# ADicksonLab/AGDIFF

Hardware: AMD Instinct MI355X
Metric: conformers/sec (whole node), GEOM-Drugs 5000-step sampling (higher is better)
Workload: dtype f16x3

## Files before the change

agdiff_amd/csrc/edge.hip:

```cpp
#include "common.hpp"

namespace {

__device__ __forceinline__ const lds_u32x4* ag_lds_base(const lds_u32x4* p, int lane) {
  const lds_u32x4* b = p + lane;
  asm volatile("" : "+v"(b));
  return b;
}

struct EncArgs {
  const float* fe_w;
  const float* fe_b;
  const float* t1;
  const float* w1_pk;
  const float* t3;
  const float* w23_pk;
  const float* w4_pk;
  const float* b4;
  const int32_t* n_dev;
  const float* e_len;
  const int32_t* e_type;
  float* out_frag;
  float* out_rows;
  const int32_t* row_index;
// ... 218 lines not shown
    pf_t1 = a.e_dst[last];
  };
  {
    const int64_t first = ((int64_t)wg * AG_CONV_WAVES + wave) * a.chunk_tiles;
    if (first * AG_TW < E) {
#pragma unroll
      for (int t = 0; t < 4; ++t) ag_load_attr(ea[t], a.e_attr, first, t, lane0);
      prefetch_meta(first, lane0);
    }
  }
  for (int64_t chunk = (int64_t)wg * AG_CONV_WAVES + wave; chunk < a.max_chunks; chunk += cstride) {
    const int64_t e_begin = chunk * (AG_TW * a.chunk_tiles);
    if (e_begin >= E) break;
    int run_t = -1;
    float carry[AG_CONV_NCH / 4];
#pragma unroll
    for (int i = 0; i < AG_CONV_NCH / 4; ++i) carry[i] = 0.0f;

    auto dest = [&](int t) -> float* {
      const int lo = a.in_ptr[t];
      return (lo >= e_begin) ? (a.agg + (size_t)t * 192) : (a.agg_first + (size_t)chunk * 192);
    };

    for (int tt = 0; tt < a.chunk_tiles; ++tt) {
      const int64_t tile = chunk * a.chunk_tiles + tt;
      const int64_t tbase = tile * AG_TW;
      if (tbase >= E) break;
      int lane = lane0;
      asm volatile("" : "+v"(lane));
      const int q = lane >> 4, col = lane & 15;
      const int my_src = pf_src;
      const float s1 = pf_s1, s2 = pf_s2;
      const int t0 = __builtin_amdgcn_readfirstlane(pf_t0);
      const int t1 = __builtin_amdgcn_readfirstlane(pf_t1);
      if (run_t >= 0 && run_t != t0) {
        float* dp = dest(run_t);
#pragma unroll
        for (int i = 0; i < AG_CONV_NCH / 4; ++i) {
          dp[16 * (4 * i + q) + col] = carry[i];
          carry[i] = 0.0f;
        }
        run_t = -1;
      }

      uint32_t xoff[4];
      f32x4 sr;
#pragma unroll
      for (int r = 0; r < 4; ++r) {
        xoff[r] = ((uint32_t)__shfl(my_src, 4 * q + r) * 192u + (uint32_t)col) * 4u;
        sr[r] = __shfl(s1, 4 * q + r);
      }
      const int ntg = t1 - t0 + 1;
      const int ipl = a.in_ptr[t0 + (lane <= ntg ? lane : ntg)];
      auto bound = [&](int i) -> int {
        return (i < 64) ? __builtin_amdgcn_readlane(ipl, i) : __builtin_amdgcn_readfirstlane(a.in_ptr[t0 + i]);
      };
      auto dest_lo = [&](int t, int lo) -> float* {
        return (lo >= e_begin) ? (a.agg + (size_t)t * 192) : (a.agg_first + (size_t)chunk * 192);
      };

      constexpr int XA = 2, XR = XA + 1;
      f32x4 xring[XR];
      float bring[XR];
      auto fetch_x = [&](int nt) {
        const char* xb = reinterpret_cast<const char*>(a.xs);
#pragma unroll
        for (int r = 0; r < 4; ++r) xring[nt % XR][r] = *reinterpret_cast<const float*>(xb + (size_t)xoff[r] + 64 * nt);
        bring[nt % XR] = a.cp.filt_b2[16 * nt + col];
      };
#pragma unroll
      for (int nt = 0; nt < XA; ++nt) fetch_x(nt);
      auto prefetch_next = [&]() {
        int64_t nxt = tile + 1;
        if (tt + 1 >= a.chunk_tiles) nxt = (chunk + cstride) * a.chunk_tiles;
        if (nxt * AG_TW < E && nxt < a.max_chunks * a.chunk_tiles) {
#pragma unroll
          for (int t = 0; t < 4; ++t) ag_load_attr(ea[t], a.e_attr, nxt, t, lane);
          prefetch_meta(nxt, lane);
        }
      };
      AgIn<MODE> hidb[6];
      {
        constexpr int WA = 1, WR = WA + 1;
        u32x4 wq[WR][2][2];
        const lds_u32x4* w1_lo = ag_lds_base(w1, lane);
        const lds_u32x4* w1_hi = ag_lds_base(w1 + 32 * 128, lane);
        auto fetch_w = [&](u32x4 (&dst)[2][2], int step) {
          const int m = step >> 2, t = step & 3;
#pragma unroll
          for (int b = 0; b < 2; ++b) {
            const int bi = t * AG_CONV_NCH + 2 * m + b;
            const lds_u32x4* wb = (bi < 32) ? w1_lo + bi * 128 : w1_hi + (bi - 32) * 128;
            dst[b][0] = wb[0];
            dst[b][1] = wb[64];
          }
        };
#pragma unroll
        for (int s0 = 0; s0 < WA; ++s0) fetch_w(wq[s0 % WR], s0);
        f32x4 hp0 = {0.f, 0.f, 0.f, 0.f}, hp1 = {0.f, 0.f, 0.f, 0.f};
#pragma unroll
        for (int m = 0; m <= AG_CONV_NCH / 2; ++m) {
          f32x4 h0 = {0.f, 0.f, 0.f, 0.f}, h1 = {0.f, 0.f, 0.f, 0.f};
          if (m < AG_CONV_NCH / 2) {
            h0 = nb0;
            h1 = nb1;
            const int mn = (m + 1) % (AG_CONV_NCH / 2);
            nb0 = ag_ld4(a.cp.filt_b1 + 32 * mn + 4 * q);
            nb1 = ag_ld4(a.cp.filt_b1 + 32 * mn + 16 + 4 * q);
          }
#pragma unroll
          for (int t = 0; t < 4; ++t) {
            const int step = m * 4 + t;
            if (m < AG_CONV_NCH / 2) {
              if (step + WA < 4 * (AG_CONV_NCH / 2)) fetch_w(wq[(step + WA) % WR], step + WA);
              ag_block_mma<MODE, false>(h0, ea[t], wq[step % WR][0]);
              ag_block_mma<MODE, false>(h1, ea[t], wq[step % WR][1]);
            }
            if (m > 0) {
              float v0 = (t < 2) ? hp0[2 * t] : hp1[2 * t - 4], v1 = (t < 2) ? hp0[2 * t + 1] : hp1[2 * t - 3];
              v0 = ag_ssp_base2(v0); v1 = ag_ssp_base2(v1);
              asm volatile("" : "+v"(v0), "+v"(v1));
              ag_cvt_pair(hidb[m - 1], 2 * t, v0, v1);
            }
            __builtin_amdgcn_sched_barrier(0);
          }
          hp0 = h0; hp1 = h1;
        }
        prefetch_next();
      }
      f32x4 m0, m1;
      {
        const int b0 = bound(0), b1 = bound(1), b2 = bound(ntg >= 2 ? 2 : 1);
#pragma unroll
        for (int r = 0; r < 4; ++r) {
          const int er = (int)tbase + 4 * q + r;
          m0[r] = (er >= b0 && er < b1) ? 1.0f : 0.0f;
          m1[r] = (ntg >= 2 && er >= b1 && er < b2) ? 1.0f : 0.0f;
        }
      }
      float* const dp0 = dest_lo(t0, bound(0));
      const bool fast = ntg <= 2;
      const bool two = ntg == 2;
      auto reduce_general = [&](f32x4 z, int nt, float& cr) {
        const bool mine = q == (nt & 3);
        float newcarry = 0.0f;
        for (int i = 0; i < ntg; ++i) {
          const int lo = bound(i), hi = bound(i + 1);
          float p = 0.0f;
#pragma unroll
          for (int r = 0; r < 4; ++r) {
            const int er = (int)tbase + 4 * q + r;
            p += ((er >= lo) && (er < hi)) ? z[r] : 0.0f;
          }
          p = ag_quarter_sum(p);
          if (i == 0) p = cr + p;
          if (i < ntg - 1) {
            float* dp = dest_lo(t0 + i, lo);
            if (mine) dp[16 * nt + col] = p;
          } else {
            newcarry = p;
          }
        }
        cr = mine ? newcarry : cr;
      };
      const u32x4* gl = reinterpret_cast<const u32x4*>(a.cp.filt_w2b_pk) + lane;
      u32x4 g[2][2];
      auto fetch_g = [&](int pair) {
#pragma unroll
        for (int b = 0; b < 2; ++b) {
          g[b][0] = gl[((2 * pair + b) * 2) * 64];
          g[b][1] = gl[((2 * pair + b) * 2 + 1) * 64];
        }
      };
      const lds_u32x4* w2a_l = ag_lds_base(w2a, lane);
      constexpr int LA = 1, LR = LA + 1;
      u32x4 w2q[LR][2];
      auto fetch_w2 = [&](int b) {
        w2q[b % LR][0] = w2a_l[(b * 2) * 64];
        w2q[b % LR][1] = w2a_l[(b * 2 + 1) * 64];
      };
#pragma unroll
      for (int b = 0; b < LA; ++b) fetch_w2(b);
      auto dense2 = [&](int nt) -> f32x4 {
        f32x4 z[1] = {{0.f, 0.f, 0.f, 0.f}};
        if (nt == 7) fetch_g(0);
        if (nt < 8) {
#pragma unroll
          for (int k = 0; k < 4; ++k) {
            const int b = nt * 4 + k;
            if (b + LA < 32) fetch_w2(b + LA);
            ag_block_mma<MODE, true>(z[0], hidb[k], w2q[b % LR]);
          }
        } else {
          ag_block_mma<MODE, true>(z[0], hidb[4], g[0]);
          ag_block_mma<MODE, true>(z[0], hidb[5], g[1]);
          if (nt + 1 < AG_CONV_NCH) fetch_g(nt + 1 - 8);
        }
        return z[0];
      };
      auto factors = [&](int nt, float& bb, f32x4& m, bool with_scale) {
        if (nt == 8) {
#pragma unroll
          for (int r = 0; r < 4; ++r) sr[r] = __shfl(s2, 4 * q + r);
        }
        bb = bring[nt % XR];
        m = with_scale ? sr * xring[nt % XR] : xring[nt % XR];
        if (nt + XA < AG_CONV_NCH) fetch_x(nt + XA);
      };
      auto run_fast = [&](auto TWO) {
        constexpr bool kTwo = decltype(TWO)::value;
        f32x4 zp = {0.f, 0.f, 0.f, 0.f}, mp = {0.f, 0.f, 0.f, 0.f};
        float bp = 0.0f;
        float p0[4], p1[4] = {0.f, 0.f, 0.f, 0.f};
        f32x4 w0 = m0 * sr, w1 = m1 * sr;
#pragma unroll
        for (int nt = 0; nt <= AG_CONV_NCH; ++nt) {
          f32x4 z = {0.f, 0.f, 0.f, 0.f}, m = {0.f, 0.f, 0.f, 0.f};
          float bb = 0.0f;
          if (nt < AG_CONV_NCH) {
            z = dense2(nt);
            factors(nt, bb, m, false);
          }
          if (nt == 9) { w0 = m0 * sr; w1 = m1 * sr; }
          if (nt > 0) {
            const int j = (nt - 1) & 3, g4 = (nt - 1) >> 2;
            f32x4 t;
#pragma unroll
            for (int r = 0; r < 4; ++r) t[r] = (zp[r] + bp) * mp[r];
            p0[j] = t[0] * w0[0];
#pragma unroll
            for (int r = 1; r < 4; ++r) p0[j] = fmaf(t[r], w0[r], p0[j]);
            if constexpr (kTwo) {
              p1[j] = t[0] * w1[0];
#pragma unroll
              for (int r = 1; r < 4; ++r) p1[j] = fmaf(t[r], w1[r], p1[j]);
            }
            if (j == 3) {
              const float r0 = carry[g4] + ag_quarter_reduce_scatter4(p0[0], p0[1], p0[2], p0[3]);
              if constexpr (kTwo) {
                dp0[16 * (4 * g4 + q) + col] = r0;
                carry[g4] = ag_quarter_reduce_scatter4(p1[0], p1[1], p1[2], p1[3]);
              } else {
                carry[g4] = r0;
              }
            }
          }
          zp = z; mp = m; bp = bb;
        }
      };
      if (fast) {
        if (two) run_fast(std::true_type{});
        else run_fast(std::false_type{});
      } else {
#pragma unroll
        for (int nt = 0; nt < AG_CONV_NCH; ++nt) {
          f32x4 z = dense2(nt), m;
          float bb;
          factors(nt, bb, m, true);
#pragma unroll
          for (int r = 0; r < 4; ++r) z[r] = (z[r] + bb) * m[r];
          reduce_general(z, nt, carry[nt >> 2]);
        }
      }
      run_t = t1;
    }
    if (run_t >= 0) {
      float* dp = dest(run_t);
#pragma unroll
      for (int i = 0; i < AG_CONV_NCH / 4; ++i) dp[16 * (4 * i + (lane0 >> 4)) + (lane0 & 15)] = carry[i];
    }
  }
}

struct HeadArgs {
  agdiff_head_params_t hp;
  const int32_t* n_dev;
  const int32_t* src;
  const int32_t* dst;
  const float* node_h;
  const float* attr_frag;
  const float* attr_rows;
  const int32_t* pos_index;
  const int32_t* mir_index;
  float* out;
  int64_t max_tiles;
};

template <int MODE>
__global__ void __launch_bounds__(64 * AG_PERSIST_WAVES, 4) k_pair_head(HeadArgs a) {
  extern __shared__ u32x4 ag_head_smem[];
  lds_u32x4* lw1 = (lds_u32x4*)ag_head_smem;
  lds_u32x4* lw2 = lw1 + 64 * 128;
  {
    const u32x4* g1 = reinterpret_cast<const u32x4*>(a.hp.w1_pk);
    const u32x4* g2 = reinterpret_cast<const u32x4*>(a.hp.w2_pk);
    ag_copy_lds(lw1, g1, 64 * 128);
    ag_copy_lds(lw2, g2, 16 * 128);
  }
  __syncthreads();
  const int lane0 = ag_lane();
  const int E = *a.n_dev;
  const int64_t stride = (int64_t)gridDim.x * AG_PERSIST_WAVES;
  const int64_t wg = (gridDim.x % 8 == 0) ? (int64_t)(blockIdx.x % 8) * (gridDim.x / 8) + blockIdx.x / 8 : (int64_t)blockIdx.x;
  for (int64_t tile = wg * AG_PERSIST_WAVES + (threadIdx.x >> 6); tile < a.max_tiles; tile += stride) {
    if (tile * AG_TW >= E) break;
    int lane = lane0;
    asm volatile("" : "+v"(lane));
    const int q = lane >> 4;
    const int64_t e = tile * AG_TW + (lane & 15);
    const bool valid = e < E;
    const int s = valid ? a.src[e] : 0, t = valid ? a.dst[e] : 0;
    const int pp = (a.pos_index && valid) ? a.pos_index[e] : 0;

    f32x4 y1[8];
    ag_init_vec<8>(y1, a.hp.b1, q);
    {
      const float* hs = a.node_h + (size_t)ag_piece_row_value(s, lane) * 128;
      const float* ht = a.node_h + (size_t)ag_piece_row_value(t, lane) * 128;
      const int64_t er = tile * AG_TW + (lane >> 2);
      const float* ar = a.attr_rows + (size_t)(er < E ? er : 0) * 128;
      const int to_op = ag_to_operand_addr(lane);
      AgIn<MODE> sl[2];
      f32x4 raw[4];
      auto fetch = [&](f32x4 (&r)[4], AgIn<MODE>& dst, int k) {
        if (k < 4) {
          ag_load_slice_pieces(r[0], r[1], hs, k, lane);
          ag_load_slice_pieces(r[2], r[3], ht, k, lane);
        } else if (a.attr_frag && a.pos_index) {
          ag_load_attr(dst, a.attr_frag, (int64_t)(pp >> 4), k - 4, q * 16 + (pp & 15));
        } else if (a.attr_frag) {
          ag_load_attr(dst, a.attr_frag, tile, k - 4, lane);
        } else {
          ag_load_slice_pieces(r[0], r[1], ar, k - 4, lane);
        }
      };
      auto finish = [&](AgIn<MODE>& dst, const f32x4 (&r)[4], int k) {
        if (k < 4) ag_cvt(ag_permute4(r[0] * r[2], to_op), ag_permute4(r[1] * r[3], to_op), dst);
        else if (!a.attr_frag) ag_cvt(ag_permute4(r[0], to_op), ag_permute4(r[1], to_op), dst);
      };
      fetch(raw, sl[0], 0);
      finish(sl[0], raw, 0);
      const lds_u32x4* lw1_lo = ag_lds_base(lw1, lane);
      const lds_u32x4* lw1_hi = ag_lds_base(lw1 + 32 * 128, lane);
#pragma unroll
      for (int k = 0; k < 8; ++k) {
        if (k + 1 < 8) fetch(raw, sl[(k + 1) & 1], k + 1);
        const lds_u32x4* wk = (k < 4) ? lw1_lo + (k * 8) * 128 : lw1_hi + ((k - 4) * 8) * 128;
        if (k & 1) ag_dense_lds<MODE, false, true, 1, 8, 1, 0>(sl, y1, wk, 0);
        else ag_dense_lds<MODE, false, true, 1, 8, 0, 0>(sl, y1, wk, 0);
        if (k + 1 < 8) finish(sl[(k + 1) & 1], raw, k + 1);
      }
    }
    ag_head_act<8>(y1, a.hp.act);
    f32x4 y2[4];
    ag_init_vec<4>(y2, a.hp.b2, q);
    {
      AgIn<MODE> y1b[4];
      ag_report_range<MODE>(ag_absmax<MODE, 8>(y1, 0.0f), a.hp.range_rows, s, valid);
      ag_cvt_tiles<MODE, 4, 0>(y1, y1b);
      ag_dense_lds<MODE, false, false, 4, 4, 0, 0>(y1b, y2, ag_lds_base(lw2, lane), 0);
    }
    ag_head_act<4>(y2, a.hp.act);
    const float o = ag_dot_vec<4>(y2, a.hp.w3, q) + a.hp.b3;
    if (valid && q == 0) {
      int l2 = lane0;
      asm volatile("" : "+v"(l2));
      const int64_t e2 = tile * AG_TW + (l2 & 15);
      a.out[a.pos_index ? (int64_t)pp : e2] = o;
      const int pm = a.pos_index ? a.mir_index[e2] : -1;
      if (pm >= 0) a.out[pm] = o;
    }
  }
}

struct RadScaleArgs {
  const float* dw[2 * AGDIFF_MAX_CONVS];
  const int32_t* rad_cnt;
  int32_t* rad_src;
  float* rad_len;
  float* out;
  int64_t rpad;
  int32_t n;
  float cutoff;
  int32_t smooth;
};
__global__ void __launch_bounds__(256) k_rad_scales(RadScaleArgs a) {
  __shared__ float seg[2 * AGDIFF_MAX_CONVS * 100];
  for (int i = threadIdx.x; i < a.n * 100; i += blockDim.x) seg[i] = a.dw[i / 100][i % 100];
  __syncthreads();
  const int64_t row = (int64_t)blockIdx.x * blockDim.x + threadIdx.x;
  if (row >= a.rpad) return;
  const int i = (int)(row / AGDIFF_RAD_STRIDE), k = (int)(row - (int64_t)i * AGDIFF_RAD_STRIDE);
  const int cnt = a.rad_cnt[i];
  if (k >= ((cnt + AG_TW - 1) / AG_TW) * AG_TW) return;
  if (k >= cnt) {
    a.rad_src[row] = i;
    a.rad_len[row] = 0.0f;
    for (int c = 0; c < a.n; ++c) a.out[(size_t)c * a.rpad + row] = 0.0f;
    return;
  }
  const float d = a.rad_len[row];
  const float C = cf_envelope(d, a.cutoff, a.smooth);
  for (int c = 0; c < a.n; ++c) a.out[(size_t)c * a.rpad + row] = cf_dist_weight(seg + c * 100, d) * C;
}

__global__ void k_zero_word(int32_t* p) {
  if (threadIdx.x == 0) *p = 0;
}

struct AttrPolyArgs {
  const float* poly_pk;
  const int32_t* type_slot;
  const int32_t* n_dev;
  const float* e_len;
  const int32_t* e_type;
  float* out_rows;
  int32_t* flags;
  int64_t max_tiles;
  int32_t num_slots;
  int32_t far_slots;
  const int32_t* type_far;
  float cutoff;
  float two_over_rc;
  float far_hi;
  float two_over_far;
};

#define AG_ATTRP_WAVES 16
#define AG_ATTRP_MAX_SLOTS 9
template <int MODE>
__global__ void __launch_bounds__(64 * AG_ATTRP_WAVES, AG_ATTRP_WAVES / 4) k_edge_attr_poly(AttrPolyArgs a) {
  extern __shared__ u32x4 ag_attrp_smem[];
  lds_u32x4* wl = (lds_u32x4*)ag_attrp_smem;
  __shared__ int wg_flagged;
  if (threadIdx.x == 0) wg_flagged = 0;
  ag_copy_lds(wl, reinterpret_cast<const u32x4*>(a.poly_pk), (a.num_slots + a.far_slots) * 8 * 128);
  __syncthreads();
  const int lane0 = ag_lane();
  const int E = *a.n_dev;
  const int64_t stride = (int64_t)gridDim.x * AG_ATTRP_WAVES;
  int my_flagged = 0;
  for (int64_t tile = (int64_t)blockIdx.x * AG_ATTRP_WAVES + (threadIdx.x >> 6); tile < a.max_tiles; tile += stride) {
    if (tile * AG_TW >= E) break;
    int lane = lane0;
    asm volatile("" : "+v"(lane));
    const int q = lane >> 4;
    const int64_t e = tile * AG_TW + (lane & 15);
    const bool valid = e < E;
    const float d = valid ? a.e_len[e] : 0.0f;
    const int ety = valid ? a.e_type[e] : 0;
    const int tslot = valid ? a.type_slot[ety] : -1;
    const int fset = (valid && a.far_slots > 0) ? a.type_far[ety] : -1;
    const bool is_nan = (__float_as_uint(d) & 0x7FFFFFFFu) > 0x7F800000u;
    const bool far = d > a.cutoff && d <= a.far_hi && tslot >= 0 && fset >= 0;
    const int slot = far ? fset : tslot;
    const bool hard = valid && (is_nan || d < 0.0f || (d > a.cutoff && !far) || tslot < 0);
    const int hard_rows = (int)(__ballot(hard) & 0xFFFFull);
    if (lane == 0) a.flags[1 + tile] = hard_rows;
    if (hard_rows) ++my_flagged;
    if (hard_rows == (int)(__ballot(valid) & 0xFFFFull)) continue;
    AgIn<MODE> phall[1], ph[1];
    ag_poly_features<MODE, 1>(far ? d - a.cutoff : d, far ? a.two_over_far : a.two_over_rc, q, phall);
    f32x4 y[8];
#pragma unroll
    for (int t = 0; t < 8; ++t) y[t] = f32x4{0.f, 0.f, 0.f, 0.f};
    const lds_u32x4* wl_l = ag_lds_base(wl, lane);
    uint64_t todo = __ballot(slot >= 0 && !hard) & 0xFFFFull;
    while (todo) {
      const int g = __builtin_amdgcn_readlane(slot, (int)__builtin_ctzll(todo));
      const bool in = slot == g && !hard;
      todo &= ~__ballot(in);
      const u32x4 zero = {0u, 0u, 0u, 0u};
      if constexpr (MODE == AG_F32) {
        ph[0].v[0] = in ? phall[0].v[0] : f32x4{0.f, 0.f, 0.f, 0.f};
        ph[0].v[1] = in ? phall[0].v[1] : f32x4{0.f, 0.f, 0.f, 0.f};
      } else {
        ph[0].hi = __builtin_bit_cast(decltype(ph[0].hi), in ? __builtin_bit_cast(u32x4, phall[0].hi) : zero);
        ph[0].lo = __builtin_bit_cast(decltype(ph[0].lo), in ? __builtin_bit_cast(u32x4, phall[0].lo) : zero);
      }
      const lds_u32x4* wg_ = wl_l + (size_t)g * (8 * 128);
      u32x4 w[8][2];
#pragma unroll
      for (int ot = 0; ot < 8; ++ot) {
        w[ot][0] = wg_[(ot * 2) * 64];
        w[ot][1] = wg_[(ot * 2 + 1) * 64];
      }
#pragma unroll
      for (int part = 0; part < AgParts<MODE>::n; ++part) {
#pragma unroll
        for (int ot = 0; ot < 8; ++ot) ag_block_mma_part<MODE, false>(y[ot], ph[0], w[ot], part);
      }
    }
    const bool ok = ag_piece_row_value(valid && !hard, lane) != 0;
    ag_store_row_pieces<8, 0>(y, a.out_rows + (size_t)(tile * AG_TW + (lane >> 2)) * 128, ok, lane);
  }
  if (lane0 == 0 && my_flagged) atomicAdd(&wg_flagged, my_flagged);
  __syncthreads();
  if (threadIdx.x == 0 && wg_flagged) atomicAdd(&a.flags[0], wg_flagged);
}

struct HeadPolyArgs {
  agdiff_head_params_t hp;
  const int32_t* n_dev;
  const int32_t* src;
  const int32_t* dst;
  const float* len;
  const float* node_h;
  const int32_t* pos_index;
  const int32_t* mir_index;
  float* out;
  int64_t max_tiles;
  float two_over_rc;
  const int32_t* seg_tile_live;
};

template <int MODE, int NKT>
__global__ void __launch_bounds__(64 * AG_PERSIST_WAVES, 4) k_pair_head_poly(HeadPolyArgs a) {
  extern __shared__ u32x4 ag_headp_smem[];
  lds_u32x4* lw1 = (lds_u32x4*)ag_headp_smem;
  lds_u32x4* lwp = lw1 + 32 * 128;
  lds_u32x4* lw2 = lwp + 8 * NKT * 128;
  {
    const u32x4* g1 = reinterpret_cast<const u32x4*>(a.hp.w1_pk);
    const u32x4* gp = reinterpret_cast<const u32x4*>(a.hp.attr_poly_pk);
    const u32x4* g2 = reinterpret_cast<const u32x4*>(a.hp.w2_pk);
    ag_copy_lds(lw1, g1, 32 * 128);
    ag_copy_lds(lwp, gp, 8 * NKT * 128);
    ag_copy_lds(lw2, g2, 16 * 128);
  }
  __syncthreads();
  const int lane0 = ag_lane();
  const int E = a.seg_tile_live ? 0 : *a.n_dev;
  const int64_t stride = (int64_t)gridDim.x * AG_PERSIST_WAVES;
  const int64_t wg = (gridDim.x % 8 == 0) ? (int64_t)(blockIdx.x % 8) * (gridDim.x / 8) + blockIdx.x / 8 : (int64_t)blockIdx.x;
  for (int64_t tile = wg * AG_PERSIST_WAVES + (threadIdx.x >> 6); tile < a.max_tiles; tile += stride) {
    int64_t live_end;
    if (a.seg_tile_live) {
      const int live = a.seg_tile_live[tile];
      if (live == 0) continue;
      live_end = tile * AG_TW + live;
    } else {
      live_end = E;
      if (tile * AG_TW >= E) break;
    }
    int lane = lane0;
    asm volatile("" : "+v"(lane));
    const int q = lane >> 4;
    const int64_t e = tile * AG_TW + (lane & 15);
    const bool valid = e < live_end;
    const int s = valid ? a.src[e] : 0, t = valid ? a.dst[e] : 0;
    const float d = valid ? a.len[e] : 0.0f;
    const int64_t pe = a.pos_index ? (valid ? (int64_t)a.pos_index[e] : 0) : e;
    const int64_t pm = (a.pos_index && valid) ? (int64_t)a.mir_index[e] : -1;

    f32x4 y1[8];
    ag_init_vec<8>(y1, a.hp.b1, q);
    {
      const float* hs = a.node_h + (size_t)ag_piece_row_value(s, lane) * 128;
      const float* ht = a.node_h + (size_t)ag_piece_row_value(t, lane) * 128;
      const int to_op = ag_to_operand_addr(lane);
      AgIn<MODE> sl[2];
      f32x4 raw[4];
      auto fetch = [&](f32x4 (&r)[4], int k) {
        ag_load_slice_pieces(r[0], r[1], hs, k, lane);
        ag_load_slice_pieces(r[2], r[3], ht, k, lane);
      };
      auto finish = [&](AgIn<MODE>& dst, const f32x4 (&r)[4]) {
        ag_cvt(ag_permute4(r[0] * r[2], to_op), ag_permute4(r[1] * r[3], to_op), dst);
      };
      fetch(raw, 0);
      finish(sl[0], raw);
      const lds_u32x4* lw1_l = ag_lds_base(lw1, lane);
#pragma unroll
      for (int k = 0; k < 4; ++k) {
        if (k + 1 < 4) fetch(raw, k + 1);
        if (k & 1) ag_dense_lds<MODE, false, true, 1, 8, 1, 0>(sl, y1, lw1_l + (k * 8) * 128, 0);
        else ag_dense_lds<MODE, false, true, 1, 8, 0, 0>(sl, y1, lw1_l + (k * 8) * 128, 0);
        if (k + 1 < 4) finish(sl[(k + 1) & 1], raw);
      }
      AgIn<MODE> ph[NKT];
      ag_poly_features<MODE, NKT>(d, a.two_over_rc, q, ph);
      ag_dense_lds<MODE, false, true, NKT, 8, 0, 0>(ph, y1, ag_lds_base(lwp, lane), 0);
    }
    ag_head_act<8>(y1, a.hp.act);
    f32x4 y2[4];
    ag_init_vec<4>(y2, a.hp.b2, q);
    {
      AgIn<MODE> y1b[4];
      ag_report_range<MODE>(ag_absmax<MODE, 8>(y1, 0.0f), a.hp.range_rows, s, valid);
      ag_cvt_tiles<MODE, 4, 0>(y1, y1b);
      ag_dense_lds<MODE, false, false, 4, 4, 0, 0>(y1b, y2, ag_lds_base(lw2, lane), 0);
    }
    ag_head_act<4>(y2, a.hp.act);
    const float o = ag_dot_vec<4>(y2, a.hp.w3, q) + a.hp.b3;
    if (valid && q == 0) {
      a.out[pe] = o;
      if (pm >= 0) a.out[pm] = o;
    }
  }
}

template <int F>
__global__ void __launch_bounds__(AG_WG) k_cfconv_aggregate(const float* __restrict__ x, const float* __restrict__ W,
                                                            const int32_t* __restrict__ in_ptr,
                                                            const int32_t* __restrict__ src, int64_t n,
                                                            float* __restrict__ out) {
  constexpr int LPE = F / 4;
  constexpr int EPI = 64 / LPE;
  const int lane = ag_lane();
  const int64_t node = (int64_t)blockIdx.x * 4 + ag_wave_in_wg();
  if (node >= n) return;
  const int lo = in_ptr[node], hi = in_ptr[node + 1];
  const int sub = lane / LPE, fl = (lane % LPE) * 4;
  f32x4 acc = {0.f, 0.f, 0.f, 0.f};
  for (int e = lo + sub; e < hi; e += EPI) {
    const f32x4 w = ag_ld4(W + (size_t)e * F + fl);
    const f32x4 xv = ag_ld4(x + (size_t)src[e] * F + fl);
    acc += w * xv;
  }
#pragma unroll
  for (int o = LPE; o < 64; o <<= 1) {
#pragma unroll
    for (int q = 0; q < 4; ++q) acc[q] += __shfl_xor(acc[q], o);
  }
  if (sub == 0) ag_st4(out + (size_t)node * F + fl, acc);
}

}

static thread_local const int32_t* g_enc_tile_flags = nullptr;

extern "C" int agdiff_edge_encoder(const agdiff_params_t* p, const int32_t* n_edges_dev, int64_t max_tiles,
                                   const float* e_len, const int32_t* e_type, float* attr_frag, float* attr_rows,
                                   const int32_t* row_index, const int32_t* pos_index, const int32_t* mir_index,
                                   void* stream) {
  if (!p || !n_edges_dev || !e_len || !e_type || (!attr_frag && !attr_rows) || max_tiles < 0 || (!pos_index != !mir_index))
    return AGDIFF_ERR_ARG;
  if (max_tiles == 0) return AGDIFF_OK;
  if (p->edge_encoder == 1) {
    if (!p->ge_offset || !p->ge_emb) return AGDIFF_ERR_ARG;
    GaussArgs g{p->ge_offset, p->ge_emb, n_edges_dev, e_len, e_type, attr_frag, attr_rows, row_index, pos_index, mir_index,
                max_tiles, p->ge_coeff * 1.44269504088896340736f};
    const dim3 grid((unsigned)((max_tiles + 3) / 4));
    ag_by_mode(p->precision, [&](auto M) { k_edge_gaussian<decltype(M)::value><<<grid, dim3(256), 0, (hipStream_t)stream>>>(g); });
    AG_CHECK_LAUNCH();
    return AGDIFF_OK;
  }
  if (p->edge_encoder != 0) return AGDIFF_ERR_ARG;
  EncArgs a{p->ee_fe_w, p->ee_fe_b, p->ee_t1, p->ee_w1_pk, p->ee_t3, p->ee_w23_pk, p->ee_w4_pk, p->ee_b4,
            n_edges_dev, e_len, e_type, attr_frag, attr_rows, row_index, pos_index, mir_index, max_tiles, g_enc_tile_flags};
  g_enc_tile_flags = nullptr;
  int64_t wgs = (max_tiles + AG_PERSIST_WAVES - 1) / AG_PERSIST_WAVES;
  if (wgs > 256) wgs = 256;
  const size_t smem = (size_t)80 * 2048;
  static std::atomic<uint64_t> attr_done{0};
  if (!ag_allow_big_lds(attr_done, smem, k_edge_encoder<AG_BF3>, k_edge_encoder<AG_F32>, k_edge_encoder<AG_H3>)) return AGDIFF_ERR_LAUNCH;
  ag_by_mode(p->precision, [&](auto M) {
    k_edge_encoder<decltype(M)::value><<<dim3((unsigned)wgs), dim3(64 * AG_PERSIST_WAVES), smem, (hipStream_t)stream>>>(a);
  });
  AG_CHECK_LAUNCH();
  return AGDIFF_OK;
}

namespace {
int launch_edge_scales(const agdiff_params_t* p, const int32_t* n_dev, int64_t max_n, const float* e_len,
                       const int32_t* pos_index, const int32_t* mir_index, float* out, int64_t epad, void* stream,
                       const int32_t* zero_slotted_types = nullptr) {
  if (max_n == 0) return AGDIFF_OK;
  ScaleArgs a;
  a.e_type = zero_slotted_types;
  a.type_slot = zero_slotted_types ? p->poly_type_slot : nullptr;
  for (int k = 0; k < p->num_convs; ++k) {
    a.dw[2 * k] = p->conv[k].dist_seg;
    a.dw[2 * k + 1] = p->conv[k].dist_seg + 100;
  }
  a.n_dev = n_dev;
  a.e_len = e_len;
  a.pos_index = pos_index;
  a.mir_index = mir_index;
  a.out = out;
  a.epad = epad;
  a.n = 2 * p->num_convs;
  a.cutoff = p->cutoff;
  a.smooth = p->smooth;
  k_edge_scales<<<dim3((unsigned)((max_n + 255) / 256)), dim3(256), 0, (hipStream_t)stream>>>(a);
  AG_CHECK_LAUNCH();
  return AGDIFF_OK;
}
}

extern "C" int agdiff_edge_scales(const agdiff_params_t* p, const agdiff_topo_t* topo, const agdiff_ws_t* ws,
                                  int32_t per_canonical_edge, void* stream) {
  if (!p || !topo || !ws || !ws->e_scale || !ws->e_len || !ws->num_edges || p->num_convs > AGDIFF_MAX_CONVS)
    return AGDIFF_ERR_ARG;
  if (per_canonical_edge && (!ws->num_canon || !ws->c_len || !ws->c_pos || !ws->c_mir)) return AGDIFF_ERR_ARG;
  const int64_t epad = ((topo->max_edges + AG_TW - 1) / AG_TW) * AG_TW;
  return launch_edge_scales(p, per_canonical_edge ? ws->num_canon : ws->num_edges, topo->max_edges,
                            per_canonical_edge ? ws->c_len : ws->e_len, per_canonical_edge ? ws->c_pos : nullptr,
                            per_canonical_edge ? ws->c_mir : nullptr, ws->e_scale, epad, stream);
}

extern "C" int agdiff_edge_scales_split(const agdiff_params_t* p, const agdiff_topo_t* topo, const agdiff_ws_t* ws,
                                        int32_t which, void* stream) {
  if (!p || !topo || !ws || p->num_convs > AGDIFF_MAX_CONVS) return AGDIFF_ERR_ARG;
  if (which == 0) {
    if (!ws->r_scale || !ws->rad_len || !ws->rad_src || !ws->rad_cnt) return AGDIFF_ERR_ARG;
    if (topo->num_nodes <= 0) return AGDIFF_OK;
    RadScaleArgs a;
    for (int k = 0; k < p->num_convs; ++k) {
      a.dw[2 * k] = p->conv[k].dist_seg;
      a.dw[2 * k + 1] = p->conv[k].dist_seg + 100;
    }
    a.rad_cnt = ws->rad_cnt;
    a.rad_src = ws->rad_src;
    a.rad_len = ws->rad_len;
    a.out = ws->r_scale;
    a.rpad = topo->num_nodes * (int64_t)AGDIFF_RAD_STRIDE;
    a.n = 2 * p->num_convs;
    a.cutoff = p->cutoff;
    a.smooth = p->smooth;
    k_rad_scales<<<dim3((unsigned)((a.rpad + 255) / 256)), dim3(256), 0, (hipStream_t)stream>>>(a);
    AG_CHECK_LAUNCH();
    return AGDIFF_OK;
  }
  if (!ws->lc_len || !ws->num_local_canon) return AGDIFF_ERR_ARG;
  if (which == 1) {
    if (!ws->l_scale || !topo->lc_ppos || !topo->lc_pmir) return AGDIFF_ERR_ARG;
    return launch_edge_scales(p, ws->num_local_canon, topo->num_local_canon, ws->lc_len, topo->lc_ppos, topo->lc_pmir,
                              ws->l_scale, ((topo->num_local_padded + AG_TW - 1) / AG_TW) * AG_TW, stream,
                              agdiff_local_poly_enabled(p, topo, ws) == 2 ? topo->lc_type : nullptr);
  }
  if (!ws->lt_scale || !topo->lc_tpos || !topo->lc_tmir) return AGDIFF_ERR_ARG;
  return launch_edge_scales(p, ws->num_local_canon, topo->num_local_canon, ws->lc_len, topo->lc_tpos, topo->lc_tmir,
                            ws->lt_scale, topo->num_local_tiles * AG_TW, stream);
}

namespace {
int launch_cfconv_fused(const agdiff_params_t* p, int32_t k, int64_t max_e, const int32_t* n_dev, const int32_t* in_ptr,
                        const int32_t* e_src, const int32_t* e_dst, const float* scales, const float* e_attr, const float* xs,
                        float* agg, float* agg_first, void* stream) {
  const int64_t max_tiles = (max_e + AG_TW - 1) / AG_TW;
  const int chunk_tiles = agdiff_conv_chunk_tiles(max_e);
  const int64_t max_chunks = (max_tiles + chunk_tiles - 1) / chunk_tiles;
  if (max_chunks == 0) return AGDIFF_OK;
  ConvArgs a;
  a.cp = p->conv[k];
  a.n_dev = n_dev;
  a.in_ptr = in_ptr;
  a.e_src = e_src;
  a.e_dst = e_dst;
  {
    const size_t epad = (size_t)max_tiles * AG_TW;
    a.scale1 = scales + (size_t)(2 * k) * epad;
    a.scale2 = scales + (size_t)(2 * k + 1) * epad;
  }
  a.e_attr = e_attr;
  a.xs = xs;
  a.agg = agg;
  a.agg_first = agg_first;
  a.max_chunks = max_chunks;
  a.chunk_tiles = chunk_tiles;
  int64_t wgs = (max_chunks + AG_CONV_WAVES - 1) / AG_CONV_WAVES;
  if (wgs > 256) wgs = 256;
  const size_t smem = (size_t)AG_CONV_LDS_BLOCKS * 2048;
  static std::atomic<uint64_t> attr_done{0};
  if (!ag_allow_big_lds(attr_done, smem, k_cfconv_fused<AG_BF3>, k_cfconv_fused<AG_F32>, k_cfconv_fused<AG_H3>)) return AGDIFF_ERR_LAUNCH;
  ag_by_mode(p->precision, [&](auto M) {
    k_cfconv_fused<decltype(M)::value><<<dim3((unsigned)wgs), dim3(64 * AG_CONV_WAVES), smem, (hipStream_t)stream>>>(a);
  });
  AG_CHECK_LAUNCH();
  return AGDIFF_OK;
}

}

extern "C" int agdiff_cfconv_fused(const agdiff_params_t* p, const agdiff_topo_t* topo, const agdiff_ws_t* ws, int32_t k,
                                   void* stream) {
  if (!p || !topo || !ws || k < 0 || k >= p->num_convs) return AGDIFF_ERR_ARG;
  ag_log_variant(ws, AGDIFF_VAR_CFCONV_FUSED);
  return launch_cfconv_fused(p, k, topo->max_edges, ws->num_edges, ws->in_ptr, ws->e_src, ws->e_dst, ws->e_scale, ws->e_attr,
                             ws->xs, ws->agg, ws->agg_first, stream);
}

extern "C" int agdiff_local_poly_enabled(const agdiff_params_t* p, const agdiff_topo_t* topo, const agdiff_ws_t* ws) {
  const bool on = p && topo && ws && !p->tune_local_poly_off && p->poly_kt >= 1 && p->poly_kt <= AGDIFF_POLY_MAX_KT &&
                  p->poly_num_slots > 0 && p->poly_num_slots <= AGDIFF_POLY_MAX_SLOTS && p->poly_type_slot && topo->lt_ptr &&
                  topo->lt_src && topo->lt_type && ws->lt_len && ws->lt_scale;
  if (!on) return 0;
  const uint64_t miss0 = (uint64_t)topo->local_type_mask[0] & ~(uint64_t)p->poly_slot_mask[0];
  const uint64_t miss1 = (uint64_t)topo->local_type_mask[1] & ~(uint64_t)p->poly_slot_mask[1];
  if (!(miss0 | miss1)) return 1;
  const uint64_t have = ((uint64_t)topo->local_type_mask[0] & (uint64_t)p->poly_slot_mask[0]) |
                        ((uint64_t)topo->local_type_mask[1] & (uint64_t)p->poly_slot_mask[1]);
  return have ? 2 : 0;
}

extern "C" int agdiff_cfconv_local(const agdiff_params_t* p, const agdiff_topo_t* topo, const agdiff_ws_t* ws, int32_t k,
                                   void* stream) {
  if (!p || !topo || !ws || k < 0 || k >= p->num_convs) return AGDIFF_ERR_ARG;
  if (topo->num_local == 0) return AGDIFF_OK;
  if (!topo->lp_ptr || !topo->lp_src || !topo->lp_dst || !ws->l_scale || !ws->l_attr_frag || !ws->agg_loc ||
      !ws->agg_first_loc || !ws->num_local_padded)
    return AGDIFF_ERR_ARG;
  ag_log_variant(ws, AGDIFF_VAR_CFCONV_LOCAL_MLP);
  return launch_cfconv_fused(p, k, topo->num_local_padded, ws->num_local_padded, topo->lp_ptr, topo->lp_src, topo->lp_dst,
                             ws->l_scale, ws->l_attr_frag, ws->xs, ws->agg_loc, ws->agg_first_loc, stream);
}

namespace {
int launch_pair_head_poly(const agdiff_params_t* p, const int32_t* n_edges_dev, int64_t max_tiles,
                          const int32_t* src, const int32_t* dst, const float* len, const float* node_h,
                          const int32_t* pos_index, const int32_t* mir_index, float* out, const int32_t* seg_tile_live,
                          int32_t* range_rows, void* stream);
}

extern "C" int agdiff_pair_head_poly(const agdiff_params_t* p, const int32_t* n_edges_dev, int64_t max_tiles,
                                     const int32_t* src, const int32_t* dst, const float* len, const float* node_h,
                                     const int32_t* pos_index, const int32_t* mir_index, float* out, void* stream) {
  if (!n_edges_dev) return AGDIFF_ERR_ARG;
  return launch_pair_head_poly(p, n_edges_dev, max_tiles, src, dst, len, node_h, pos_index, mir_index, out, nullptr, nullptr, stream);
}

extern "C" int agdiff_pair_head_poly_rows(const agdiff_params_t* p, const agdiff_topo_t* topo, const agdiff_ws_t* ws,
                                          int32_t parity, void* stream) {
  if (!p || !topo || !ws || !ws->canon_counter || !ws->inv_r) return AGDIFF_ERR_ARG;
  const int64_t tiles = (topo->max_edges - topo->num_local + AG_TW - 1) / AG_TW + 1;
  return launch_pair_head_poly(p, ws->canon_counter + (parity & 1), tiles, ws->c_src, ws->c_dst, ws->c_len, ws->h, ws->c_pos,
                               ws->c_mir, ws->inv_r, nullptr, ws->range_rows, stream);
}

namespace {
int launch_pair_head_poly(const agdiff_params_t* p, const int32_t* n_edges_dev, int64_t max_tiles,
                          const int32_t* src, const int32_t* dst, const float* len, const float* node_h,
                          const int32_t* pos_index, const int32_t* mir_index, float* out, const int32_t* seg_tile_live,
                          int32_t* range_rows, void* stream) {
  if (!p || !src || !dst || !len || !node_h || !out || max_tiles < 0 || (!pos_index != !mir_index))
    return AGDIFF_ERR_ARG;
  if (p->poly_kt < 1 || p->poly_kt > AGDIFF_POLY_MAX_KT || !p->head_global.attr_poly_pk) return AGDIFF_ERR_ARG;
  if (max_tiles == 0) return AGDIFF_OK;
  HeadPolyArgs a;
  a.hp = p->head_global;
  if (range_rows) a.hp.range_rows = range_rows;
  a.seg_tile_live = seg_tile_live;
  a.n_dev = n_edges_dev;
  a.src = src;
  a.dst = dst;
  a.len = len;
  a.node_h = node_h;
  a.pos_index = pos_index;
  a.mir_index = mir_index;
  a.out = out;
  a.max_tiles = max_tiles;
  a.two_over_rc = 2.0f / p->cutoff;
  int64_t wgs = (max_tiles + AG_PERSIST_WAVES - 1) / AG_PERSIST_WAVES;
  if (wgs > 256) wgs = 256;
  const size_t smem = (size_t)(48 + 8 * p->poly_kt) * 2048;
  static std::atomic<uint64_t> attr_done{0};
#define AG_HEADP_KERNELS(M) k_pair_head_poly<M, 1>, k_pair_head_poly<M, 2>, k_pair_head_poly<M, 3>, k_pair_head_poly<M, 4>
  if (!ag_allow_big_lds(attr_done, (size_t)(48 + 8 * AGDIFF_POLY_MAX_KT) * 2048, AG_HEADP_KERNELS(AG_BF3), AG_HEADP_KERNELS(AG_F32),
                        AG_HEADP_KERNELS(AG_H3)))
    return AGDIFF_ERR_LAUNCH;
#undef AG_HEADP_KERNELS
  const dim3 grid((unsigned)wgs), block(64 * AG_PERSIST_WAVES);
  hipStream_t st = (hipStream_t)stream;
  ag_by_mode(p->precision, [&](auto MODE_) {
    constexpr int MODE = decltype(MODE_)::value;
    switch (p->poly_kt) {
      case 1: k_pair_head_poly<MODE, 1><<<grid, block, smem, st>>>(a); break;
      case 2: k_pair_head_poly<MODE, 2><<<grid, block, smem, st>>>(a); break;
      case 3: k_pair_head_poly<MODE, 3><<<grid, block, smem, st>>>(a); break;
      default: k_pair_head_poly<MODE, 4><<<grid, block, smem, st>>>(a); break;
    }
  });
  AG_CHECK_LAUNCH();
  return AGDIFF_OK;
}
}

extern "C" int agdiff_local_edge_rows(const agdiff_params_t* p, const agdiff_topo_t* topo, const agdiff_ws_t* ws, void* stream) {
  if (!p || !topo || !ws) return AGDIFF_ERR_ARG;
  if (topo->num_local == 0) return AGDIFF_OK;
  if (!ws->l_attr_rows || !ws->lc_len || !ws->num_local_canon || !topo->lc_type || topo->num_local_canon <= 0) return AGDIFF_ERR_ARG;
  const int64_t ctiles = (topo->num_local_canon + AG_TW - 1) / AG_TW;
  const bool poly = !p->tune_attr_poly_off && p->edge_encoder == 0 && p->poly_kt == 1 && p->poly_num_slots > 0 &&
                    p->poly_num_slots <= AG_ATTRP_MAX_SLOTS && p->attr_poly_typed_pk && p->poly_type_slot && ws->enc_flags;
  if (p->attr_poly_far_slots < 0 ||
      (p->attr_poly_far_slots > 0 && (p->poly_num_slots + p->attr_poly_far_slots > AG_ATTRP_MAX_SLOTS || !p->attr_poly_far_set ||
                                      !(p->attr_poly_far_hi > p->cutoff))))
    return AGDIFF_ERR_ARG;
  if (!poly)
    return agdiff_edge_encoder(p, ws->num_local_canon, ctiles, ws->lc_len, topo->lc_type, nullptr, ws->l_attr_rows, nullptr,
                               nullptr, nullptr, stream);
  hipStream_t st = (hipStream_t)stream;
  k_zero_word<<<1, 64, 0, st>>>(ws->enc_flags);
  AG_CHECK_LAUNCH();
  AttrPolyArgs a;
  a.poly_pk = p->attr_poly_typed_pk;
  a.type_slot = p->poly_type_slot;
  a.n_dev = ws->num_local_canon;
  a.e_len = ws->lc_len;
  a.e_type = topo->lc_type;
  a.out_rows = ws->l_attr_rows;
  a.flags = ws->enc_flags;
  a.max_tiles = ctiles;
  a.num_slots = p->poly_num_slots;
  a.far_slots = poly ? p->attr_poly_far_slots : 0;
  a.type_far = p->attr_poly_far_set;
  a.cutoff = p->cutoff;
  a.two_over_rc = 2.0f / p->cutoff;
  a.far_hi = a.far_slots > 0 ? p->attr_poly_far_hi : p->cutoff;
  a.two_over_far = a.far_slots > 0 ? 2.0f / (p->attr_poly_far_hi - p->cutoff) : 0.0f;
  int64_t wgs = (ctiles + AG_ATTRP_WAVES - 1) / AG_ATTRP_WAVES;
  if (wgs > 256) wgs = 256;
  const size_t smem = (size_t)(p->poly_num_slots + a.far_slots) * 8 * 2048;
  static std::atomic<uint64_t> attr_done{0};
  if (!ag_allow_big_lds(attr_done, (size_t)AG_ATTRP_MAX_SLOTS * 8 * 2048, k_edge_attr_poly<AG_BF3>, k_edge_attr_poly<AG_F32>,
                        k_edge_attr_poly<AG_H3>))
    return AGDIFF_ERR_LAUNCH;
  ag_by_mode(p->precision_local, [&](auto M) {
    k_edge_attr_poly<decltype(M)::value><<<dim3((unsigned)wgs), dim3(64 * AG_ATTRP_WAVES), smem, st>>>(a);
  });
  AG_CHECK_LAUNCH();
  ag_log_variant(ws, AGDIFF_VAR_ATTR_POLY);
  g_enc_tile_flags = ws->enc_flags;
  const int rc = agdiff_edge_encoder(p, ws->num_local_canon, ctiles, ws->lc_len, topo->lc_type, nullptr, ws->l_attr_rows,
                                     nullptr, nullptr, nullptr, stream);
  g_enc_tile_flags = nullptr;
  return rc;
}

extern "C" int agdiff_pair_head(const agdiff_head_params_t* hp, const int32_t* n_edges_dev, int64_t max_tiles,
                                const int32_t* src, const int32_t* dst, const float* node_h, const float* attr_frag,
                                const float* attr_rows, const int32_t* pos_index, const int32_t* mir_index, float* out,
                                void* stream) {
  if (!hp || !n_edges_dev || !src || !dst || !node_h || (!attr_frag == !attr_rows) || !out || max_tiles < 0 ||
      (!pos_index != !mir_index))
    return AGDIFF_ERR_ARG;
  if (max_tiles == 0) return AGDIFF_OK;
  HeadArgs a;
  a.hp = *hp;
  a.n_dev = n_edges_dev;
  a.src = src;
  a.dst = dst;
  a.node_h = node_h;
  a.attr_frag = attr_frag;
  a.attr_rows = attr_rows;
  a.pos_index = pos_index;
  a.mir_index = mir_index;
  a.out = out;
  a.max_tiles = max_tiles;
  int64_t wgs = (max_tiles + AG_PERSIST_WAVES - 1) / AG_PERSIST_WAVES;
  if (wgs > 256) wgs = 256;
  const size_t smem = (size_t)80 * 2048;
  static std::atomic<uint64_t> attr_done{0};
  if (!ag_allow_big_lds(attr_done, smem, k_pair_head<AG_BF3>, k_pair_head<AG_F32>, k_pair_head<AG_H3>)) return AGDIFF_ERR_LAUNCH;
  ag_by_mode(hp->precision, [&](auto M) {
    k_pair_head<decltype(M)::value><<<dim3((unsigned)wgs), dim3(64 * AG_PERSIST_WAVES), smem, (hipStream_t)stream>>>(a);
  });
  AG_CHECK_LAUNCH();
  return AGDIFF_OK;
}

extern "C" int agdiff_cfconv_aggregate(const float* x, const float* W, const int32_t* in_ptr, const int32_t* src,
                                       int64_t num_nodes, int32_t F, float* out, void* stream) {
  if (!x || !W || !in_ptr || !src || !out || num_nodes < 0) return AGDIFF_ERR_ARG;
  if (F != 64 && F != 128) return AGDIFF_ERR_LIMIT;
  if (num_nodes == 0) return AGDIFF_OK;
  dim3 grid((unsigned)((num_nodes + 3) / 4));
  if (F == 128)
    k_cfconv_aggregate<128><<<grid, dim3(AG_WG), 0, (hipStream_t)stream>>>(x, W, in_ptr, src, num_nodes, out);
  else
    k_cfconv_aggregate<64><<<grid, dim3(AG_WG), 0, (hipStream_t)stream>>>(x, W, in_ptr, src, num_nodes, out);
  AG_CHECK_LAUNCH();
  return AGDIFF_OK;
}
```

Baseline: 174.8.

## Software-pipeline next tile's index and node-feature loads in pair head kernels

Restructures the persistent tile loops in k_pair_head and k_pair_head_poly so the src/dst/len indices and first slice of node features for the next tile are fetched during the current tile's dense layers. Sched barriers pin the loads ahead of the LDS matmuls to hide global-memory latency. Out-of-range lanes read a clamped index, and pos/mir indices are loaded later. It also removes the unused seg_tile_live path from the poly head. This raises register pressure and adds scheduling constraints in exchange for latency hiding.

New measurement: 175.7 (median of 6 runs). About the same (+0.5%).

```diff
diff --git a/agdiff_amd/csrc/edge.hip b/agdiff_amd/csrc/edge.hip
--- a/agdiff_amd/csrc/edge.hip
+++ b/agdiff_amd/csrc/edge.hip
@@ -544,49 +544,72 @@
   const int E = *a.n_dev;
   const int64_t stride = (int64_t)gridDim.x * AG_PERSIST_WAVES;
   const int64_t wg = (gridDim.x % 8 == 0) ? (int64_t)(blockIdx.x % 8) * (gridDim.x / 8) + blockIdx.x / 8 : (int64_t)blockIdx.x;
-  for (int64_t tile = wg * AG_PERSIST_WAVES + (threadIdx.x >> 6); tile < a.max_tiles; tile += stride) {
-    if (tile * AG_TW >= E) break;
+  int64_t tile = wg * AG_PERSIST_WAVES + __builtin_amdgcn_readfirstlane((int)(threadIdx.x >> 6));
+  if (tile >= a.max_tiles || tile * AG_TW >= E) return;
+  auto entries = [&](int64_t tl, int ln, int& s, int& t) {
+    const unsigned e = (unsigned)(tl * AG_TW) + (ln & 15);
+    const bool valid = e < (unsigned)E;
+    const unsigned ec = valid ? e : (unsigned)E - 1;
+    const int ls = a.src[ec], lt = a.dst[ec];
+    s = valid ? ls : 0;
+    t = valid ? lt : 0;
+  };
+  auto attr_row = [&](int64_t tl, int ln) {
+    const unsigned er = (unsigned)(tl * AG_TW) + (ln >> 2);
+    return er < (unsigned)E ? er : 0u;
+  };
+  int s, t;
+  entries(tile, lane0, s, t);
+  int rs = ag_piece_row_value(s, lane0), rt = ag_piece_row_value(t, lane0);
+  unsigned ra = attr_row(tile, lane0);
+  f32x4 raw[4];
+  ag_load_slice_pieces(raw[0], raw[1], a.node_h + (size_t)rs * 128, 0, lane0);
+  ag_load_slice_pieces(raw[2], raw[3], a.node_h + (size_t)rt * 128, 0, lane0);
+  for (;;) {
     int lane = lane0;
     asm volatile("" : "+v"(lane));
     const int q = lane >> 4;
-    const int64_t e = tile * AG_TW + (lane & 15);
-    const bool valid = e < E;
-    const int s = valid ? a.src[e] : 0, t = valid ? a.dst[e] : 0;
-    const int pp = (a.pos_index && valid) ? a.pos_index[e] : 0;
+    const unsigned e = (unsigned)(tile * AG_TW) + (lane & 15);
+    const bool valid = e < (unsigned)E;
+    const int64_t next = tile + stride;
+    const bool more = next < a.max_tiles && next * AG_TW < E;
+    const int64_t ptile = more ? next : tile;
+    int ns, nt;
+    int pp = 0;
+    if (a.attr_frag && a.pos_index) {
+      const int lp = a.pos_index[valid ? e : (unsigned)E - 1];
+      pp = valid ? lp : 0;
+    }
 
     f32x4 y1[8];
     ag_init_vec<8>(y1, a.hp.b1, q);
     {
-      const float* hs = a.node_h + (size_t)ag_piece_row_value(s, lane) * 128;
-      const float* ht = a.node_h + (size_t)ag_piece_row_value(t, lane) * 128;
-      const int64_t er = tile * AG_TW + (lane >> 2);
-      const float* ar = a.attr_rows + (size_t)(er < E ? er : 0) * 128;
       const int to_op = ag_to_operand_addr(lane);
       AgIn<MODE> sl[2];
-      f32x4 raw[4];
       auto fetch = [&](f32x4 (&r)[4], AgIn<MODE>& dst, int k) {
         if (k < 4) {
-          ag_load_slice_pieces(r[0], r[1], hs, k, lane);
-          ag_load_slice_pieces(r[2], r[3], ht, k, lane);
+          ag_load_slice_pieces(r[0], r[1], a.node_h + (size_t)rs * 128, k, lane);
+          ag_load_slice_pieces(r[2], r[3], a.node_h + (size_t)rt * 128, k, lane);
         } else if (a.attr_frag && a.pos_index) {
           ag_load_attr(dst, a.attr_frag, (int64_t)(pp >> 4), k - 4, q * 16 + (pp & 15));
         } else if (a.attr_frag) {
           ag_load_attr(dst, a.attr_frag, tile, k - 4, lane);
         } else {
-          ag_load_slice_pieces(r[0], r[1], ar, k - 4, lane);
+          ag_load_slice_pieces(r[0], r[1], a.attr_rows + (size_t)ra * 128, k - 4, lane);
         }
       };
       auto finish = [&](AgIn<MODE>& dst, const f32x4 (&r)[4], int k) {
         if (k < 4) ag_cvt(ag_permute4(r[0] * r[2], to_op), ag_permute4(r[1] * r[3], to_op), dst);
         else if (!a.attr_frag) ag_cvt(ag_permute4(r[0], to_op), ag_permute4(r[1], to_op), dst);
       };
-      fetch(raw, sl[0], 0);
       finish(sl[0], raw, 0);
       const lds_u32x4* lw1_lo = ag_lds_base(lw1, lane);
       const lds_u32x4* lw1_hi = ag_lds_base(lw1 + 32 * 128, lane);
 #pragma unroll
       for (int k = 0; k < 8; ++k) {
         if (k + 1 < 8) fetch(raw, sl[(k + 1) & 1], k + 1);
+        __builtin_amdgcn_sched_barrier(0);
+        if (k == 3) entries(ptile, lane, ns, nt);
         const lds_u32x4* wk = (k < 4) ? lw1_lo + (k * 8) * 128 : lw1_hi + ((k - 4) * 8) * 128;
         if (k & 1) ag_dense_lds<MODE, false, true, 1, 8, 1, 0>(sl, y1, wk, 0);
         else ag_dense_lds<MODE, false, true, 1, 8, 0, 0>(sl, y1, wk, 0);
@@ -596,22 +619,31 @@
     ag_head_act<8>(y1, a.hp.act);
     f32x4 y2[4];
     ag_init_vec<4>(y2, a.hp.b2, q);
+    int po = 0, pm = -1;
+    if (a.pos_index) {
+      const unsigned ec = valid ? e : (unsigned)E - 1;
+      po = a.pos_index[ec];
+      pm = a.mir_index[ec];
+    }
     {
       AgIn<MODE> y1b[4];
       ag_report_range<MODE>(ag_absmax<MODE, 8>(y1, 0.0f), a.hp.range_rows, s, valid);
       ag_cvt_tiles<MODE, 4, 0>(y1, y1b);
+      rs = ag_piece_row_value(ns, lane), rt = ag_piece_row_value(nt, lane), ra = attr_row(ptile, lane);
+      ag_load_slice_pieces(raw[0], raw[1], a.node_h + (size_t)rs * 128, 0, lane);
+      ag_load_slice_pieces(raw[2], raw[3], a.node_h + (size_t)rt * 128, 0, lane);
+      __builtin_amdgcn_sched_barrier(0);
       ag_dense_lds<MODE, false, false, 4, 4, 0, 0>(y1b, y2, ag_lds_base(lw2, lane), 0);
     }
     ag_head_act<4>(y2, a.hp.act);
     const float o = ag_dot_vec<4>(y2, a.hp.w3, q) + a.hp.b3;
     if (valid && q == 0) {
-      int l2 = lane0;
-      asm volatile("" : "+v"(l2));
-      const int64_t e2 = tile * AG_TW + (l2 & 15);
-      a.out[a.pos_index ? (int64_t)pp : e2] = o;
-      const int pm = a.pos_index ? a.mir_index[e2] : -1;
+      a.out[a.pos_index ? (int64_t)po : (int64_t)e] = o;
       if (pm >= 0) a.out[pm] = o;
     }
+    if (!more) break;
+    tile = next;
+    s = ns;
   }
 }
 
@@ -753,7 +785,6 @@
   float* out;
   int64_t max_tiles;
   float two_over_rc;
-  const int32_t* seg_tile_live;
 };
 
 template <int MODE, int NKT>
@@ -772,50 +803,58 @@
   }
   __syncthreads();
   const int lane0 = ag_lane();
-  const int E = a.seg_tile_live ? 0 : *a.n_dev;
+  const int E = *a.n_dev;
   const int64_t stride = (int64_t)gridDim.x * AG_PERSIST_WAVES;
   const int64_t wg = (gridDim.x % 8 == 0) ? (int64_t)(blockIdx.x % 8) * (gridDim.x / 8) + blockIdx.x / 8 : (int64_t)blockIdx.x;
-  for (int64_t tile = wg * AG_PERSIST_WAVES + (threadIdx.x >> 6); tile < a.max_tiles; tile += stride) {
-    int64_t live_end;
-    if (a.seg_tile_live) {
-      const int live = a.seg_tile_live[tile];
-      if (live == 0) continue;
-      live_end = tile * AG_TW + live;
-    } else {
-      live_end = E;
-      if (tile * AG_TW >= E) break;
-    }
+  int64_t tile = wg * AG_PERSIST_WAVES + __builtin_amdgcn_readfirstlane((int)(threadIdx.x >> 6));
+  if (tile >= a.max_tiles || tile * AG_TW >= E) return;
+  auto entries = [&](int64_t tl, int ln, int& s, int& t, float& d) {
+    const unsigned e = (unsigned)(tl * AG_TW) + (ln & 15);
+    const bool valid = e < (unsigned)E;
+    const unsigned ec = valid ? e : (unsigned)E - 1;
+    const int ls = a.src[ec], lt = a.dst[ec];
+    const float ld = a.len[ec];
+    s = valid ? ls : 0;
+    t = valid ? lt : 0;
+    d = valid ? ld : 0.0f;
+  };
+  int s, t;
+  float d;
+  entries(tile, lane0, s, t, d);
+  int rs = ag_piece_row_value(s, lane0), rt = ag_piece_row_value(t, lane0);
+  f32x4 raw[4];
+  auto fetch = [&](f32x4 (&r)[4], int k, int lane) {
+    ag_load_slice_pieces(r[0], r[1], a.node_h + (size_t)rs * 128, k, lane);
+    ag_load_slice_pieces(r[2], r[3], a.node_h + (size_t)rt * 128, k, lane);
+  };
+  fetch(raw, 0, lane0);
+  constexpr bool PIN = MODE != AG_BF3;
+  for (;;) {
     int lane = lane0;
     asm volatile("" : "+v"(lane));
     const int q = lane >> 4;
-    const int64_t e = tile * AG_TW + (lane & 15);
-    const bool valid = e < live_end;
-    const int s = valid ? a.src[e] : 0, t = valid ? a.dst[e] : 0;
-    const float d = valid ? a.len[e] : 0.0f;
-    const int64_t pe = a.pos_index ? (valid ? (int64_t)a.pos_index[e] : 0) : e;
-    const int64_t pm = (a.pos_index && valid) ? (int64_t)a.mir_index[e] : -1;
+    const unsigned e = (unsigned)(tile * AG_TW) + (lane & 15);
+    const bool valid = e < (unsigned)E;
+    const int64_t next = tile + stride;
+    const bool more = next < a.max_tiles && next * AG_TW < E;
+    int ns, nt;
+    float nd;
+    entries(more ? next : tile, lane, ns, nt, nd);
 
     f32x4 y1[8];
     ag_init_vec<8>(y1, a.hp.b1, q);
     {
-      const float* hs = a.node_h + (size_t)ag_piece_row_value(s, lane) * 128;
-      const float* ht = a.node_h + (size_t)ag_piece_row_value(t, lane) * 128;
       const int to_op = ag_to_operand_addr(lane);
       AgIn<MODE> sl[2];
-      f32x4 raw[4];
-      auto fetch = [&](f32x4 (&r)[4], int k) {
-        ag_load_slice_pieces(r[0], r[1], hs, k, lane);
-        ag_load_slice_pieces(r[2], r[3], ht, k, lane);
-      };
       auto finish = [&](AgIn<MODE>& dst, const f32x4 (&r)[4]) {
         ag_cvt(ag_permute4(r[0] * r[2], to_op), ag_permute4(r[1] * r[3], to_op), dst);
       };
-      fetch(raw, 0);
       finish(sl[0], raw);
       const lds_u32x4* lw1_l = ag_lds_base(lw1, lane);
 #pragma unroll
       for (int k = 0; k < 4; ++k) {
-        if (k + 1 < 4) fetch(raw, k + 1);
+        if (k + 1 < 4) fetch(raw, k + 1, lane);
+        if constexpr (PIN) __builtin_amdgcn_sched_barrier(0);
         if (k & 1) ag_dense_lds<MODE, false, true, 1, 8, 1, 0>(sl, y1, lw1_l + (k * 8) * 128, 0);
         else ag_dense_lds<MODE, false, true, 1, 8, 0, 0>(sl, y1, lw1_l + (k * 8) * 128, 0);
         if (k + 1 < 4) finish(sl[(k + 1) & 1], raw);
@@ -827,18 +866,30 @@
     ag_head_act<8>(y1, a.hp.act);
     f32x4 y2[4];
     ag_init_vec<4>(y2, a.hp.b2, q);
+    int pp = 0, pm = -1;
+    if (a.pos_index) {
+      const unsigned ec = valid ? e : (unsigned)E - 1;
+      pp = a.pos_index[ec];
+      pm = a.mir_index[ec];
+    }
     {
       AgIn<MODE> y1b[4];
       ag_report_range<MODE>(ag_absmax<MODE, 8>(y1, 0.0f), a.hp.range_rows, s, valid);
       ag_cvt_tiles<MODE, 4, 0>(y1, y1b);
+      rs = ag_piece_row_value(ns, lane), rt = ag_piece_row_value(nt, lane);
+      fetch(raw, 0, lane);
+      if constexpr (PIN) __builtin_amdgcn_sched_barrier(0);
       ag_dense_lds<MODE, false, false, 4, 4, 0, 0>(y1b, y2, ag_lds_base(lw2, lane), 0);
     }
     ag_head_act<4>(y2, a.hp.act);
     const float o = ag_dot_vec<4>(y2, a.hp.w3, q) + a.hp.b3;
     if (valid && q == 0) {
-      a.out[pe] = o;
+      a.out[a.pos_index ? (int64_t)pp : (int64_t)e] = o;
       if (pm >= 0) a.out[pm] = o;
     }
+    if (!more) break;
+    tile = next;
+    s = ns, d = nd;
   }
 }
 
@@ -1052,15 +1103,14 @@
 namespace {
 int launch_pair_head_poly(const agdiff_params_t* p, const int32_t* n_edges_dev, int64_t max_tiles,
                           const int32_t* src, const int32_t* dst, const float* len, const float* node_h,
-                          const int32_t* pos_index, const int32_t* mir_index, float* out, const int32_t* seg_tile_live,
-                          int32_t* range_rows, void* stream);
+                          const int32_t* pos_index, const int32_t* mir_index, float* out, int32_t* range_rows, void* stream);
 }
 
 extern "C" int agdiff_pair_head_poly(const agdiff_params_t* p, const int32_t* n_edges_dev, int64_t max_tiles,
                                      const int32_t* src, const int32_t* dst, const float* len, const float* node_h,
                                      const int32_t* pos_index, const int32_t* mir_index, float* out, void* stream) {
   if (!n_edges_dev) return AGDIFF_ERR_ARG;
-  return launch_pair_head_poly(p, n_edges_dev, max_tiles, src, dst, len, node_h, pos_index, mir_index, out, nullptr, nullptr, stream);
+  return launch_pair_head_poly(p, n_edges_dev, max_tiles, src, dst, len, node_h, pos_index, mir_index, out, nullptr, stream);
 }
 
 extern "C" int agdiff_pair_head_poly_rows(const agdiff_params_t* p, const agdiff_topo_t* topo, const agdiff_ws_t* ws,
@@ -1068,14 +1118,13 @@
   if (!p || !topo || !ws || !ws->canon_counter || !ws->inv_r) return AGDIFF_ERR_ARG;
   const int64_t tiles = (topo->max_edges - topo->num_local + AG_TW - 1) / AG_TW + 1;
   return launch_pair_head_poly(p, ws->canon_counter + (parity & 1), tiles, ws->c_src, ws->c_dst, ws->c_len, ws->h, ws->c_pos,
-                               ws->c_mir, ws->inv_r, nullptr, ws->range_rows, stream);
+                               ws->c_mir, ws->inv_r, ws->range_rows, stream);
 }
 
 namespace {
 int launch_pair_head_poly(const agdiff_params_t* p, const int32_t* n_edges_dev, int64_t max_tiles,
                           const int32_t* src, const int32_t* dst, const float* len, const float* node_h,
-                          const int32_t* pos_index, const int32_t* mir_index, float* out, const int32_t* seg_tile_live,
-                          int32_t* range_rows, void* stream) {
+                          const int32_t* pos_index, const int32_t* mir_index, float* out, int32_t* range_rows, void* stream) {
   if (!p || !src || !dst || !len || !node_h || !out || max_tiles < 0 || (!pos_index != !mir_index))
     return AGDIFF_ERR_ARG;
   if (p->poly_kt < 1 || p->poly_kt > AGDIFF_POLY_MAX_KT || !p->head_global.attr_poly_pk) return AGDIFF_ERR_ARG;
@@ -1083,7 +1132,6 @@
   HeadPolyArgs a;
   a.hp = p->head_global;
   if (range_rows) a.hp.range_rows = range_rows;
-  a.seg_tile_live = seg_tile_live;
   a.n_dev = n_edges_dev;
   a.src = src;
   a.dst = dst;
```
